# buaacyw/MeshAnything

Measured on NVIDIA H100. Metric: face-tokens/sec (350M, 800-face cap), higher is better.
Workload: dtype f16 weights/activations, f32 accumulate

## Files before the change

### meshanything_b200/csrc/api.cu

```cuda
#include <stdarg.h>
#include <stdlib.h>
#include <stdio.h>
#include <string.h>

#include <atomic>
#include <map>
#include <mutex>
#include <vector>

#include "canon.cuh"
#include "internal.h"

namespace ma {

static thread_local char g_err[512] = "";
static std::atomic<unsigned long long> g_launches{0};

void set_error(const char* fmt, ...) {
  va_list ap;
  va_start(ap, fmt);
  vsnprintf(g_err, sizeof(g_err), fmt, ap);
  va_end(ap);
}
void count_launch(int n) { g_launches += (unsigned long long)n; }
bool check_launch(const char* what) {
  cudaError_t e = cudaPeekAtLastError();
  if (e != cudaSuccess) {
    set_error("%s: %s", what, cudaGetErrorString(e));
    cudaGetLastError();
    return false;
  }
  return true;
}

static inline size_t align_up(size_t x, size_t a = 256) { return (x + a - 1) / a * a; }

constexpr int PREFILL_SEQS = 8;

struct DecWs {
  float* hres;
  __half *x16, *qkv, *attn16, *y16, *f16, *logits, *lastx16;
  int* nkeys;
  SeqState s;
  int* all_done;
  void* attn_scratch;
  size_t attn_scratch_bytes;
  void* attn_scratch_pre;
  size_t attn_scratch_pre_bytes;
  void* fast;
  void* tc_scratch;
  size_t total;
};

static DecWs carve(void* base, int B, int tmax, int vocab) {
  DecWs w;
  const size_t rows = (size_t)std::max(B, PREFIX * std::min(B, PREFILL_SEQS));
  size_t off = 0;
  auto take = [&](size_t bytes) {
    void* p = base ? (void*)((char*)base + off) : nullptr;
    off += align_up(bytes);
    return p;
  };
  w.hres = (float*)take(rows * HID * 4);
  w.x16 = (__half*)take(rows * HID * 2);
  w.qkv = (__half*)take(rows * QKV * 2);
  w.attn16 = (__half*)take(rows * HID * 2);
  w.y16 = (__half*)take(rows * HID * 2);
  w.f16 = (__half*)take(rows * FFN * 2);
  w.logits = (__half*)take((size_t)B * vocab * 2);
  w.lastx16 = (__half*)take((size_t)B * HID * 2);
  w.nkeys = (int*)take(rows * 4);
  w.s.pos = (int*)take((size_t)B * 4);
  w.s.gen = (int*)take((size_t)B * 4);
  w.s.tok = (int*)take((size_t)B * 4);
  w.s.finished = (int*)take((size_t)B * 4);
  w.s.lens = (int*)take((size_t)B * 4);
  w.s.sid = (int*)take((size_t)B * 4);
  w.all_done = (int*)take(256);
  w.attn_scratch_bytes = attention_scratch_bytes((int)B, NHEAD, tmax);
  w.attn_scratch = take(w.attn_scratch_bytes);
  w.attn_scratch_pre_bytes = attention_scratch_bytes(PREFIX * std::min(B, PREFILL_SEQS), NHEAD, PREFIX);
  w.attn_scratch_pre = take(w.attn_scratch_pre_bytes);
  w.fast = take(fast_workspace_bytes());
  w.tc_scratch = take(linear_ws_scratch_bytes());
  w.total = off;
  return w;
}

static inline __half* kv_layer(void* kv, int layer, int which, int B, long T) {
  return (__half*)kv + ((size_t)(layer * 2 + which) * B) * NHEAD * T * HD;
}

static const bool g_no_stream_attn = [] {
  const char* e = getenv("MA_B200_NO_STREAM_ATTN");
  return e && e[0] == '1';
}();

static const bool g_no_pdl = [] {
  const char* e = getenv("MA_B200_NO_PDL");
  return e && e[0] == '1';
}();

static int dec_linear(bool tc, const DecWs& ws, const void* W, const void* b, const __half* x, int ldx, __half* y, int ldy,
                      int M, int N, int K, int epi, cudaStream_t st, bool pdl = false) {
  if (tc) {
    const bool tiled_ok = M >= 64 && linear_tc_supported(M, N, K, ldx, ldy, x, W, y);
    const bool ws_ok = M <= 128 && linear_ws_supported(M, N, K, ldx, x, W);
    if (ws_ok && (linear_ws_mode() || !tiled_ok || K > 1024))
      return launch_linear_ws((const __half*)W, (const __half*)b, x, ldx, y, ldy, M, N, K, epi, ws.tc_scratch, st, pdl);
    if (tiled_ok) return launch_linear_tc((const __half*)W, (const __half*)b, x, ldx, y, ldy, M, N, K, epi, st);
  }
  return launch_linear((const __half*)W, (const __half*)b, x, ldx, y, ldy, M, N, K, epi, st);
}

static int run_layers(const ma_decoder_weights* w, const DecWs& ws, void* kv, int B, long T, int M, int rows_per_slot,
                      int slot0, int max_keys, cudaStream_t st, bool tc = false) {
  void* scratch = rows_per_slot > 1 ? ws.attn_scratch_pre : ws.attn_scratch;
  const bool pdl = tc && rows_per_slot == 1 && !g_no_pdl;
  for (int L = 0; L < w->n_layers; L++) {
    __half* kc = kv_layer(kv, L, 0, B, T) + (size_t)slot0 * NHEAD * T * HD;
    __half* vc = kv_layer(kv, L, 1, B, T) + (size_t)slot0 * NHEAD * T * HD;
    if (dec_linear(tc, ws, w->wqkv[L], w->bqkv[L], ws.x16, HID, ws.qkv, QKV, M, QKV, HID, MA_EPI_NONE, st, pdl)) return 1;
    if (rows_per_slot == 1 && !g_no_stream_attn) {
      if (launch_attention_decode(ws.qkv, QKV, kc, vc, T, ws.nkeys, max_keys, M, 0.125f, ws.attn16, HID, scratch, pdl,
                                  st)) return 1;
    } else {
      if (launch_kv_append(ws.qkv, M, rows_per_slot, ws.nkeys, kc, vc, T, st)) return 1;
      if (launch_attention(ws.qkv, QKV, kc, vc, T, NHEAD, rows_per_slot, nullptr, ws.nkeys, max_keys, M, 0.125f,
                           ws.attn16, HID, scratch, st)) return 1;
    }
    if (dec_linear(tc, ws, w->wo[L], w->bo[L], ws.attn16, HID, ws.y16, HID, M, HID, HID, MA_EPI_NONE, st, pdl)) return 1;
    if (launch_layernorm(ws.hres, ws.y16, w->ln1g[L], w->ln1b[L], MA_LN_EPS, M, HID, ws.hres, ws.x16, st, pdl)) return 1;
    if (dec_linear(tc, ws, w->w1[L], w->b1[L], ws.x16, HID, ws.f16, FFN, M, FFN, HID, MA_EPI_RELU, st, pdl)) return 1;
    if (dec_linear(tc, ws, w->w2[L], w->b2[L], ws.f16, FFN, ws.y16, HID, M, HID, FFN, MA_EPI_NONE, st, pdl)) return 1;
    if (launch_layernorm(ws.hres, ws.y16, w->ln2g[L], w->ln2b[L], MA_LN_EPS, M, HID, ws.hres, ws.x16, st, pdl)) return 1;
  }
  return 0;
}

struct GraphKey {
  const void *w, *kv, *ws, *out_ids, *forced, *logits_out;
  unsigned long long whash;
  int B, tmax, max_new, bucket, flags, do_sample, top_k, eos, pad, mode, ws_mode;
  float top_p;
  unsigned long long seed;
  bool operator<(const GraphKey& o) const { return memcmp(this, &o, sizeof(GraphKey)) < 0; }
};
static std::map<GraphKey, cudaGraphExec_t> g_graphs;
static std::map<cudaGraphExec_t, unsigned long long> g_graph_launches;
static cudaStream_t g_stream = nullptr;
static int* g_flag_host = nullptr;
static cudaEvent_t g_ev_in = nullptr, g_ev_out = nullptr, g_ev_flag = nullptr;

static int g_device = -1;
static std::mutex g_mu;

static int ensure_globals() {
  int dev = -1;
  if (cudaGetDevice(&dev) != cudaSuccess) {
    set_error("cudaGetDevice: %s", cudaGetErrorString(cudaGetLastError()));
    return 1;
  }
  if (g_device >= 0 && dev != g_device) {
    set_error("ma_decode_generate was first used on device %d; this process now runs on device %d "
              "(one process per GPU)", g_device, dev);
    return 1;
  }
  if (!g_stream) {
    if (cudaStreamCreateWithFlags(&g_stream, cudaStreamNonBlocking) != cudaSuccess ||
        cudaHostAlloc((void**)&g_flag_host, 64, cudaHostAllocDefault) != cudaSuccess ||
        cudaEventCreateWithFlags(&g_ev_in, cudaEventDisableTiming) != cudaSuccess ||
        cudaEventCreateWithFlags(&g_ev_out, cudaEventDisableTiming) != cudaSuccess ||
        cudaEventCreateWithFlags(&g_ev_flag, cudaEventDisableTiming) != cudaSuccess) {
      set_error("cannot create stream/events: %s", cudaGetErrorString(cudaGetLastError()));
      return 1;
    }
    g_device = dev;
  }
  return 0;
}


static int enqueue_batched_step(const ma_decoder_weights* w, const DecWs& ws, void* kv, int B, long T, int max_keys,
                                const SampleArgs& sa, cudaStream_t s, bool tc) {
  if (launch_embed_tokens(w, ws.s, B, ws.hres, ws.x16, ws.nkeys, s)) return 1;
  if (run_layers(w, ws, kv, B, T, B, 1, 0, max_keys, s, tc)) return 1;
  if (dec_linear(tc, ws, w->lm_head, nullptr, ws.x16, HID, ws.logits, w->vocab, B, w->vocab, HID, MA_EPI_NONE, s,
                 tc && !g_no_pdl)) return 1;
  return launch_sample(sa, s);
}

static inline bool use_tc(int B, int do_sample, int flags) { return B > 1 && (do_sample || (flags & MA_GEN_TC)); }

static unsigned long long weights_hash(const ma_decoder_weights* w) {
  unsigned long long h = 1469598103934665603ull;
  const unsigned char* pb = (const unsigned char*)w;
  for (size_t q = 0; q < sizeof(ma_decoder_weights); q++) h = (h ^ pb[q]) * 1099511628211ull;
  return h;
}

template <class F>
static int launch_cached_graph(const GraphKey& key, cudaStream_t st, F&& enqueue) {
  auto it = g_graphs.find(key);
  if (it == g_graphs.end()) {
    cudaGraph_t graph = nullptr;
    if (cudaStreamBeginCapture(st, cudaStreamCaptureModeThreadLocal) != cudaSuccess) {
      set_error("cudaStreamBeginCapture: %s", cudaGetErrorString(cudaGetLastError()));
      return 1;
    }
    const unsigned long long before = g_launches.load();
    int erc = enqueue(st);
    const unsigned long long per_step = g_launches.load() - before;
    cudaError_t ce = cudaStreamEndCapture(st, &graph);
    if (erc || ce != cudaSuccess || !graph) {
      if (!erc) set_error("cudaStreamEndCapture: %s", cudaGetErrorString(ce));
      cudaGetLastError();
      return 1;
    }
    cudaGraphExec_t exec = nullptr;
    ce = cudaGraphInstantiate(&exec, graph, 0);
    cudaGraphDestroy(graph);
    if (ce != cudaSuccess) {
      set_error("cudaGraphInstantiate: %s", cudaGetErrorString(ce));
      return 1;
    }
    if (g_graphs.size() > 64) {
      for (auto& kvp : g_graphs) cudaGraphExecDestroy(kvp.second);
      g_graphs.clear();
      g_graph_launches.clear();
    }
    it = g_graphs.emplace(key, exec).first;
    g_launches -= per_step;
    g_graph_launches[exec] = per_step;
  }
  if (cudaGraphLaunch(it->second, st) != cudaSuccess) {
    set_error("cudaGraphLaunch: %s", cudaGetErrorString(cudaGetLastError()));
    return 1;
  }
  g_launches += g_graph_launches[it->second];
  return 0;
}

static void fill_sample_args(SampleArgs& sa, const ma_decoder_weights* w, const DecWs& ws, int B, int max_new,
                             const ma_sampling* sampling, int eos_id, int pad_id, int32_t* out_ids) {
  memset(&sa, 0, sizeof(sa));
  sa.logits = ws.logits; sa.vocab = w->vocab; sa.B = B; sa.max_new = max_new; sa.eos_id = eos_id; sa.pad_id = pad_id;
  sa.do_sample = sampling ? sampling->do_sample : 0;
  sa.top_k = sampling ? sampling->top_k : 0;
  sa.top_p = sampling ? sampling->top_p : 1.0f;
  sa.seed = sampling ? sampling->seed : 0;
  sa.s = ws.s; sa.out_ids = out_ids;
}

static int check_decode_args(const char* who, const ma_decoder_weights* w, int B, int tmax, int max_new) {
  if (w->n_layers > MA_MAX_LAYERS || w->vocab > 8195 + 61) {
    set_error("%s: n_layers=%d / vocab=%d unsupported", who, w->n_layers, w->vocab);
    return 1;
  }
  if (B <= 0 || max_new <= 0 || PREFIX + max_new > tmax) {
    set_error("%s: B=%d, tmax=%d < 257 + max_new=%d", who, B, tmax, max_new);
    return 1;
  }
  if (PREFIX + max_new + 2 > w->npos) {
    set_error("%s: sequence of %d exceeds %d learned positions", who, PREFIX + max_new, w->npos - 2);
    return 1;
  }
  return 0;
}

}

using namespace ma;

extern "C" {

int ma_abi_version(void) { return MA_ABI_VERSION; }
const char* ma_last_error(void) { return g_err; }
unsigned long long ma_launch_count(void) { return g_launches.load(); }

int ma_linear_f16(const void* W, const void* bias, const void* x, int ldx, void* y, int ldy, int M, int N, int K,
                  int epilogue, void* stream) {
  return launch_linear((const __half*)W, (const __half*)bias, (const __half*)x, ldx, (__half*)y, ldy, M, N, K,
                       epilogue, (cudaStream_t)stream);
}

size_t ma_linear_ws_scratch_bytes(void) { return linear_ws_scratch_bytes(); }
void ma_linear_ws_set_mode(int cluster) { linear_ws_set_mode(cluster); }

int ma_linear_ws_f16(const void* W, const void* bias, const void* x, int ldx, void* y, int ldy, int M, int N, int K,
                     int epilogue, void* scratch, void* stream) {
  return launch_linear_ws((const __half*)W, (const __half*)bias, (const __half*)x, ldx, (__half*)y, ldy, M, N, K,
                          epilogue, scratch, (cudaStream_t)stream);
}

int ma_layernorm(const float* x, const void* res16, const float* gamma, const float* beta, float eps, int M, int W,
                 float* out32, void* out16, void* stream) {
  return launch_layernorm(x, (const __half*)res16, gamma, beta, eps, M, W, out32, (__half*)out16,
                          (cudaStream_t)stream);
}

size_t ma_attention_scratch_bytes(int M, int H, int max_keys) { return attention_scratch_bytes(M, H, max_keys); }

int ma_attention_f16(const void* q, int ldq, const void* K, const void* V, long T, int H, const int* slots,
                     const int* nkeys, int max_keys, int M, float scale, void* out, int ldo, void* scratch,
                     void* stream) {
  if (M > 65535) {
    set_error("ma_attention_f16: M=%d exceeds 65535 rows per call", M);
    return 1;
  }
  return launch_attention((const __half*)q, ldq, (const __half*)K, (const __half*)V, T, H, 1, slots, nkeys, max_keys, M,
                          scale, (__half*)out, ldo, scratch, (cudaStream_t)stream);
}

int ma_attention_decode_f16(const void* qkv, int ldq, void* K, void* V, long T, const int* nkeys, int max_keys, int M,
                            float scale, void* out, int ldo, void* scratch, void* stream) {
  if (!qkv || !K || !V || !nkeys || !out || !scratch || M < 1 || max_keys < 1 || max_keys > T || ldq < 3 * HID) {
    set_error("ma_attention_decode_f16: bad arguments (M=%d, max_keys=%d, T=%ld, ldq=%d)", M, max_keys, T, ldq);
    return 1;
  }
  return launch_attention_decode((const __half*)qkv, ldq, (__half*)K, (__half*)V, T, nkeys, max_keys, M, scale,
                                 (__half*)out, ldo, scratch, false, (cudaStream_t)stream);
}

int ma_sample_tokens(const void* logits, int B, int vocab, const ma_sampling* sampling, int32_t* out_tokens,
                     int32_t* out_support, void* stream) {
  if (!logits || !out_tokens || B < 1 || vocab < 1) {
    set_error("ma_sample_tokens: bad arguments");
    return 1;
  }
  SampleArgs sa;
  memset(&sa, 0, sizeof(sa));
  sa.logits = (const __half*)logits; sa.vocab = vocab; sa.B = B; sa.max_new = 1; sa.eos_id = -1; sa.pad_id = -1;
  sa.do_sample = sampling ? sampling->do_sample : 0;
  sa.top_k = sampling ? sampling->top_k : 0;
  sa.top_p = sampling ? sampling->top_p : 1.0f;
  sa.seed = sampling ? sampling->seed : 0;
  sa.first = 1; sa.token_out = out_tokens; sa.support_out = out_support;
  return launch_sample(sa, (cudaStream_t)stream);
}

size_t ma_kv_cache_bytes(int n_layers, int B, int tmax) {
  return (size_t)n_layers * 2 * B * NHEAD * (size_t)tmax * HD * sizeof(__half);
}

size_t ma_decoder_workspace_bytes(int B, int tmax) { return carve(nullptr, B, tmax, 8195 + 61).total; }

int ma_decode_generate(const ma_decoder_weights* w, const float* prefix, int B, int tmax, int max_new,
                       const ma_sampling* sampling, int eos_id, int pad_id, void* kv, void* ws_, int32_t* out_ids,
                       int32_t* out_lens, const int32_t* forced_ids, void* logits_out, int flags, void* stream) {
  if (!w || !prefix || !kv || !ws_ || !out_ids || B <= 0 || max_new <= 0) {
    set_error("ma_decode_generate: bad arguments");
    return 1;
  }
  if (check_decode_args("ma_decode_generate", w, B, tmax, max_new)) return 1;
  std::lock_guard<std::mutex> lock(g_mu);
  if (ensure_globals()) return 1;
  cudaStream_t user = (cudaStream_t)stream;
  cudaStream_t st = g_stream;
  cudaEventRecord(g_ev_in, user);
  cudaStreamWaitEvent(st, g_ev_in, 0);

  const long T = tmax;
  DecWs ws = carve(ws_, B, tmax, 8195 + 61);
  cudaMemsetAsync(ws.attn_scratch, 0, ws.attn_scratch_bytes, st);
  cudaMemsetAsync(ws.attn_scratch_pre, 0, ws.attn_scratch_pre_bytes, st);
  cudaMemsetAsync(ws.fast, 0, fast_workspace_bytes(), st);
  if (launch_fill_i32(out_ids, pad_id, (long)B * max_new, st)) return 1;

  SampleArgs sa;
  fill_sample_args(sa, w, ws, B, max_new, sampling, eos_id, pad_id, out_ids);
  sa.first = 1; sa.forced = forced_ids; sa.logits_out = (__half*)logits_out;
  sa.all_done = ws.all_done;

  const bool tc = use_tc(B, sa.do_sample, flags);
  if (tc) cudaMemsetAsync(ws.tc_scratch, 0, linear_ws_scratch_bytes(), st);
  const bool fast = (B == 1) && !(flags & MA_GEN_NO_FAST);
  if (fast) sa.nkeys_next = fast_nkeys_ptr(ws.fast);

  for (int b0 = 0; b0 < B; b0 += PREFILL_SEQS) {
    const int nb = std::min(PREFILL_SEQS, B - b0), M = nb * PREFIX;
    if (launch_embed_prefix(w, prefix + (size_t)b0 * PREFIX * HID, nb, ws.hres, ws.x16, ws.nkeys, st)) return 1;
    if (run_layers(w, ws, kv, B, T, M, PREFIX, b0, PREFIX, st, tc)) return 1;
    if (launch_gather_rows(ws.x16, HID, PREFIX - 1, PREFIX, nb, ws.lastx16 + (size_t)b0 * HID, st)) return 1;
  }
  if (dec_linear(tc, ws, w->lm_head, nullptr, ws.lastx16, HID, ws.logits, w->vocab, B, w->vocab, HID, MA_EPI_NONE, st))
    return 1;
  if (launch_sample(sa, st)) return 1;
  sa.first = 0;
  sa.nkeys_next = nullptr;


  const bool use_graph = !(flags & MA_GEN_NO_GRAPH);
  const bool early = !(flags & MA_GEN_NO_EARLY_EXIT) && !forced_ids;
  const int CHECK_EVERY = 64;
  const unsigned long long whash = use_graph ? weights_hash(w) : 0;
  bool flag_pending = false;
  int rc = 0;
  for (int i = 1; i < max_new && rc == 0; i++) {
    const int ctx = PREFIX + i;
// ... 193 lines not shown
```

### meshanything_b200/csrc/attention_stream.cu

```cuda
#include "canon.cuh"
#include "internal.h"

namespace ma {

constexpr int AS_SLOTS = 3;
constexpr int AS_TEAM = 256;
constexpr int AS_THREADS = 32 + AS_TEAM;
constexpr int AS_PART = 66;
constexpr int AS_MERGE_BLOCK = 29;

struct AttnStreamSmem {
  __half ring[AS_SLOTS][MA_ATTN_CHUNK * HD];
  float red[8][65];
  float pst[AS_MERGE_BLOCK * AS_PART];
  float wgt[64];
  float mst[64];
  float wmax[8];
  uint64_t full[AS_SLOTS], empty[AS_SLOTS];
  int last;
};
static_assert(2 * (sizeof(AttnStreamSmem) + 1024) <= 233472, "two CTAs of attention_stream_kernel per SM");

struct AttnStreamArgs {
  const __half* q;
  int ldq;
  __half* K;
  __half* V;
  long T;
  const int* nkeys;
  __half* out;
  int ldo;
  float* part;
  int* counters;
  int M, max_chunks;
  int cps, nseg;
  float scale;
};

__device__ __forceinline__ void team_bar() { asm volatile("bar.sync 1, %0;" ::"n"(AS_TEAM) : "memory"); }
__device__ __forceinline__ void mbar_arrive(uint64_t* bar) {
  asm volatile("mbarrier.arrive.shared::cta.b64 _, [%0];" ::"r"(smem_u32(bar)) : "memory");
}

struct AsItem {
  int m, h, c0, c1, n, nk, nch;
};
__device__ __forceinline__ bool as_item(const AttnStreamArgs& a, int w, AsItem& it) {
  const int g = w % a.nseg, h = (w / a.nseg) % NHEAD;
  it.m = w / (a.nseg * NHEAD);
  it.h = h;
  it.nk = __ldcg(a.nkeys + it.m);
  it.n = min(it.nk, a.max_chunks * MA_ATTN_CHUNK);
  it.nch = (it.n + MA_ATTN_CHUNK - 1) / MA_ATTN_CHUNK;
  it.c0 = g * a.cps;
  it.c1 = min(it.nch, it.c0 + a.cps);
  return it.c0 < it.c1;
}

__global__ void __launch_bounds__(AS_THREADS, 2) attention_stream_kernel(AttnStreamArgs a) {
  extern __shared__ __align__(128) unsigned char smem_raw[];
  AttnStreamSmem& sm = *reinterpret_cast<AttnStreamSmem*>(smem_raw);
  const int tid = threadIdx.x, warp = tid >> 5, lane = tid & 31;
  const int nitems = a.nseg * NHEAD * a.M;

  if (tid == 0) {
    for (int s = 0; s < AS_SLOTS; s++) {
      mbar_init(&sm.full[s], 1);
      mbar_init(&sm.empty[s], 1);
    }
    mbar_fence_init();
  }
  __syncthreads();

  if (warp == 0) {
    if (lane != 0) return;
    int u = 0;
    for (int w = blockIdx.x; w < nitems; w += gridDim.x) {
      AsItem it;
      if (!as_item(a, w, it)) continue;
      for (int c = it.c0; c < it.c1; c++) {
        const int len = min(MA_ATTN_CHUNK, it.n - c * MA_ATTN_CHUNK);
        const int old = (it.nk == it.n) ? min(len, (it.n - 1) - c * MA_ATTN_CHUNK) : len;
        const long base = (((long)it.m * NHEAD + it.h) * a.T + (long)c * MA_ATTN_CHUNK) * HD;
#pragma unroll
        for (int kv = 0; kv < 2; kv++, u++) {
          const int s = u % AS_SLOTS;
          if (u >= AS_SLOTS) mbar_wait(&sm.empty[s], ((u / AS_SLOTS) & 1) ^ 1);
          if (old > 0) {
            mbar_expect_tx(&sm.full[s], (uint32_t)old * HD * 2);
            bulk_g2s(sm.ring[s], (kv ? a.V : a.K) + base, (uint32_t)old * HD * 2, &sm.full[s]);
          } else {
            mbar_arrive(&sm.full[s]);
          }
        }
      }
    }
    return;
  }

  const int wt = warp - 1, tl = tid - 32;
  const int grp = lane >> 3, li = lane & 7;
  pdl_wait();
  pdl_trigger();
  int u = 0;
  for (int w = blockIdx.x; w < nitems; w += gridDim.x) {
    AsItem it;
    if (!as_item(a, w, it)) continue;
    const int m = it.m, h = it.h, nch = it.nch;
    const __half* qrow = a.q + (long)m * a.ldq + h * HD + 8 * li;
    const uint4 qp = *reinterpret_cast<const uint4*>(qrow);
    float* part = a.part + (((long)m * NHEAD + h) * a.max_chunks) * AS_PART;

    for (int c = it.c0; c < it.c1; c++, u += 2) {
      const int sk = u % AS_SLOTS, sv = (u + 1) % AS_SLOTS;
      const int len = min(MA_ATTN_CHUNK, it.n - c * MA_ATTN_CHUNK);
      const int cur = (it.nk == it.n) ? (it.n - 1) - c * MA_ATTN_CHUNK : -1;
      uint4 kcur = make_uint4(0, 0, 0, 0), vcur = kcur;
      const bool own_cur = cur >= 0 && cur < MA_ATTN_CHUNK && (4 * wt + grp) == (cur & 31);
      if (own_cur) {
        kcur = *reinterpret_cast<const uint4*>(qrow + HID);
        vcur = *reinterpret_cast<const uint4*>(qrow + 2 * HID);
        const long dst = (((long)m * NHEAD + h) * a.T + (long)c * MA_ATTN_CHUNK + cur) * HD + 8 * li;
        *reinterpret_cast<uint4*>(a.K + dst) = kcur;
        *reinterpret_cast<uint4*>(a.V + dst) = vcur;
      }
      const int rho_c = own_cur ? (cur >> 5) : -1;
      const __half* ks = sm.ring[sk];
      const __half* vs = sm.ring[sv];
      mbar_wait(&sm.full[sk], (u / AS_SLOTS) & 1);

      float pr[8];
#pragma unroll
      for (int rho = 0; rho < 8; rho++) {
        const int r = 32 * rho + 4 * wt + grp;
        uint4 x = *reinterpret_cast<const uint4*>(ks + r * HD + 8 * li);
        if (rho == rho_c) x = kcur;
        pr[rho] = dot8(qp, x, 0.0f);
      }
#pragma unroll
      for (int sft = 4; sft >= 1; sft >>= 1) {
        const bool up = (li & sft) != 0;
#pragma unroll
        for (int t = 0; t < sft; t++) {
          const float mine = up ? pr[t + sft] : pr[t];
          const float other = up ? pr[t] : pr[t + sft];
          pr[t] = fadd(mine, __shfl_xor_sync(0xffffffffu, other, sft));
        }
      }
      const float s_own = fmul(pr[0], a.scale);
      const bool own_valid = 32 * li + 4 * wt + grp < len;
      const float lmax = warp_max(own_valid ? s_own : -INFINITY);
      if (lane == 0) sm.wmax[wt] = lmax;
      team_bar();
      if (tl == 0) mbar_arrive(&sm.empty[sk]);
      float cmax = sm.wmax[0];
#pragma unroll
      for (int w2 = 1; w2 < 8; w2++) cmax = fmaxf(cmax, sm.wmax[w2]);
      const float e_own = own_valid ? ma_exp(fsub(s_own, cmax)) : 0.0f;
      float l = 0.0f, o[8];
#pragma unroll
      for (int t = 0; t < 8; t++) o[t] = 0.0f;
      mbar_wait(&sm.full[sv], ((u + 1) / AS_SLOTS) & 1);
#pragma unroll
      for (int rho = 0; rho < 8; rho++) {
        const int r = 32 * rho + 4 * wt + grp;
        const float e = __shfl_sync(0xffffffffu, e_own, (lane & 24) | rho);
        if (r < len) {
          l = fadd(l, e);
          uint4 x = *reinterpret_cast<const uint4*>(vs + r * HD + 8 * li);
          if (rho == rho_c) x = vcur;
          pv8(__float2half_rn(e), x, o);
        }
      }
      l = fadd(l, __shfl_xor_sync(0xffffffffu, l, 16));
      l = fadd(l, __shfl_xor_sync(0xffffffffu, l, 8));
#pragma unroll
      for (int t = 0; t < 8; t++) {
        o[t] = fadd(o[t], __shfl_xor_sync(0xffffffffu, o[t], 16));
        o[t] = fadd(o[t], __shfl_xor_sync(0xffffffffu, o[t], 8));
      }
      if (grp == 0) {
#pragma unroll
        for (int t = 0; t < 8; t++) sm.red[wt][8 * li + t] = o[t];
        if (li == 0) sm.red[wt][64] = l;
      }
      team_bar();
      if (tl == 0) mbar_arrive(&sm.empty[sv]);
      if (tl < 65) {
        float x[8];
#pragma unroll
        for (int w2 = 0; w2 < 8; w2++) x[w2] = sm.red[w2][tl];
        const float rsum = fadd(fadd(fadd(x[0], x[1]), fadd(x[2], x[3])), fadd(fadd(x[4], x[5]), fadd(x[6], x[7])));
        if (nch == 1) {
          sm.pst[tl] = rsum;
        } else {
          part[c * AS_PART + (tl < 64 ? tl : 65)] = rsum;
          if (tl == 64) part[c * AS_PART + 64] = cmax;
        }
      }
    }

    if (nch == 1) {
      team_bar();
      if (tl < 64) a.out[(long)m * a.ldo + h * HD + tl] = __float2half_rn(__fdiv_rn(sm.pst[tl], sm.pst[64]));
      team_bar();
      continue;
    }
    __threadfence();
    team_bar();
    const int nseg_row = (nch + a.cps - 1) / a.cps;
    if (nseg_row > 1) {
      if (tl == 0) {
        int* cnt = a.counters + (long)m * NHEAD + h;
        const int prev = atomicAdd(cnt, 1);
        const int last = (prev == nseg_row - 1);
        if (last) *cnt = 0;
        sm.last = last;
      }
      team_bar();
      const int last = sm.last;
      team_bar();
      if (!last) continue;
      __threadfence();
    }
    const bool single = nch <= AS_MERGE_BLOCK;
    if (!single) {
      for (int t = tl; t < nch; t += AS_TEAM) sm.mst[t] = __ldcg(part + t * AS_PART + 64);
      team_bar();
      float Mx = -INFINITY;
      for (int cc = 0; cc < nch; cc++) Mx = fmaxf(Mx, sm.mst[cc]);
      for (int t = tl; t < nch; t += AS_TEAM) sm.wgt[t] = ma_exp(fsub(sm.mst[t], Mx));
    }
    float Lsum = 0.0f, O = 0.0f;
    for (int c0 = 0; c0 < nch; c0 += AS_MERGE_BLOCK) {
      const int nb = min(AS_MERGE_BLOCK, nch - c0), nw = nb * AS_PART;
      for (int t = tl; t < nw; t += AS_TEAM) sm.pst[t] = __ldcg(part + (long)c0 * AS_PART + t);
      team_bar();
      if (single) {
        float Mx = -INFINITY;
        for (int cc = 0; cc < nch; cc++) Mx = fmaxf(Mx, sm.pst[cc * AS_PART + 64]);
        for (int t = tl; t < nch; t += AS_TEAM) sm.wgt[t] = ma_exp(fsub(sm.pst[t * AS_PART + 64], Mx));
        team_bar();
      }
      if (tl < 64) {
        for (int cc = 0; cc < nb; cc++) {
          const float wc = sm.wgt[c0 + cc];
          Lsum = ffma(sm.pst[cc * AS_PART + 65], wc, Lsum);
          O = ffma(sm.pst[cc * AS_PART + tl], wc, O);
        }
      }
      team_bar();
    }
    if (tl < 64) a.out[(long)m * a.ldo + h * HD + tl] = __float2half_rn(__fdiv_rn(O, Lsum));
  }
}

static int g_as_ctas = 0;

int launch_attention_decode(const __half* qkv, int ldq, __half* K, __half* V, long T, const int* nkeys, int max_keys,
                            int M, float scale, __half* out, int ldo, void* scratch, bool pdl, cudaStream_t st) {
  if (M <= 0) return 0;
  if (!g_as_ctas) {
    int dev = 0, sms = 0;
    cudaGetDevice(&dev);
    cudaDeviceGetAttribute(&sms, cudaDevAttrMultiProcessorCount, dev);
    cudaFuncSetAttribute(attention_stream_kernel, cudaFuncAttributeMaxDynamicSharedMemorySize,
                         (int)sizeof(AttnStreamSmem));
    g_as_ctas = 2 * (sms > 0 ? sms : 132);
  }
  const int chunks = (max_keys + MA_ATTN_CHUNK - 1) / MA_ATTN_CHUNK;
  AttnStreamArgs a;
  a.q = qkv; a.ldq = ldq; a.K = K; a.V = V; a.T = T; a.nkeys = nkeys; a.out = out; a.ldo = ldo;
  a.counters = reinterpret_cast<int*>(scratch);
  const size_t coff = ((size_t)M * NHEAD * sizeof(int) + 255) & ~(size_t)255;
  a.part = reinterpret_cast<float*>(reinterpret_cast<char*>(scratch) + coff);
  a.M = M; a.max_chunks = chunks; a.scale = scale;
  {
    long best = -1;
    int best_cps = 1;
    for (int cps = 1; cps <= chunks; cps++) {
      const int nseg = (chunks + cps - 1) / cps;
      const long items = (long)nseg * NHEAD * M;
      const long cost = ((items + g_as_ctas - 1) / g_as_ctas) * (long)(min(cps, chunks) + 1);
      if (best < 0 || cost <= best) { best = cost; best_cps = cps; }
    }
    a.cps = best_cps;
    a.nseg = (chunks + a.cps - 1) / a.cps;
  }
  const long nitems = (long)a.nseg * NHEAD * M;
  cudaLaunchConfig_t cfg = {};
  cfg.gridDim = dim3((unsigned)min((long)g_as_ctas, nitems));
  cfg.blockDim = dim3(AS_THREADS);
  cfg.dynamicSmemBytes = sizeof(AttnStreamSmem);
  cfg.stream = st;
  cudaLaunchAttribute at[1];
  at[0].id = cudaLaunchAttributeProgrammaticStreamSerialization;
  at[0].val.programmaticStreamSerializationAllowed = 1;
  cfg.attrs = at;
  cfg.numAttrs = pdl ? 1 : 0;
  cudaLaunchKernelEx(&cfg, attention_stream_kernel, a);
  count_launch();
  return check_launch("attention_stream_kernel") ? 0 : 1;
}

}
```

### meshanything_b200/csrc/decode_fast.cu

```cuda
#include "canon.cuh"
#include "internal.h"

namespace ma {

int launch_attention_ex(const __half* q, int ldq, const __half* K, const __half* V, long T, int H, int rows_per_slot,
                        const int* slots, const int* nkeys, int max_keys, int M, float scale, __half* out, int ldo,
                        void* scratch, int decode_prefetch, bool pdl, cudaStream_t st);

constexpr int FG_THREADS = 256;
constexpr int FG_WARPS = 8;

enum { MODE_QKV = 0, MODE_OUT = 1, MODE_FC1 = 2, MODE_FC2 = 3, MODE_LM = 4 };

struct FastWs {
  float hresA[HID];
  float hresB[HID];
  __half q[HID];
  __half attn16[HID];
  __half y16[HID];
  __half f16[FFN];
  __half logits[8256];
  float cand_val[256];
  int cand_idx[256];
  int counter;
  int nkeys;
  alignas(256) unsigned char attn_scratch[256];
};

struct FastArgs {
  const __half* W;
  const __half* bias;
  int N, rows_per_cta;
  const float* hres_in;
  const __half* y16_in;
  const float *gamma, *beta;
  const __half* x16_in;
  float* hres_out;
  int embed;
  const float *extra, *tok_pos, *cond, *pos_table;
  const __half* tok_table;
  SeqState s;
  __half* out16;
  __half *kc, *vc;
  long T;
  FastWs* ws;
  int do_argmax;
  int max_new, eos_id, pad_id;
  int32_t* out_ids;
  const int32_t* forced;
  __half* logits_out;
  int* all_done;
  int vocab;
};

template <int K>
struct alignas(128) FastSmemHdr {
  uint64_t bar[FG_WARPS];
  float red[8];
  float bval[FG_WARPS];
  int bidx[FG_WARPS];
  int last;
  alignas(16) __half xs[K];
};

template <int K, int MODE>
__global__ void __launch_bounds__(FG_THREADS) fast_gemv_kernel(FastArgs a) {
  extern __shared__ __align__(128) unsigned char smem_raw[];
  FastSmemHdr<K>& sh = *reinterpret_cast<FastSmemHdr<K>*>(smem_raw);
  __half* sw = reinterpret_cast<__half*>(smem_raw + sizeof(FastSmemHdr<K>));
  __half* sb = sw + (size_t)a.rows_per_cta * K;
  const int tid = threadIdx.x, warp = tid >> 5, lane = tid & 31;

  if (MODE != MODE_QKV) pdl_trigger();

  const int row0 = blockIdx.x * a.rows_per_cta;
  const int nrows = max(0, min(a.rows_per_cta, a.N - row0));
  const int base = nrows / FG_WARPS, rem = nrows % FG_WARPS;
  const int wr0 = warp * base + min(warp, rem);
  const int wn = base + (warp < rem ? 1 : 0);

  if (lane == 0) {
    mbar_init(&sh.bar[warp], 1);
    mbar_fence_init();
  }
  __syncwarp();
  if (lane == 0 && wn > 0) {
    mbar_expect_tx(&sh.bar[warp], (uint32_t)wn * K * 2);
    bulk_g2s(sw + (size_t)wr0 * K, a.W + (size_t)(row0 + wr0) * K, (uint32_t)wn * K * 2, &sh.bar[warp]);
  }
  if (a.bias)
    for (int i = tid; i < nrows; i += FG_THREADS) sb[i] = a.bias[row0 + i];
  float4 ln_g, ln_b, cond;
  if (MODE == MODE_QKV && a.embed) {
    cond = *reinterpret_cast<const float4*>(a.cond + HID + 4 * tid);
  } else if (MODE == MODE_QKV || MODE == MODE_FC1 || MODE == MODE_LM) {
    ln_g = *reinterpret_cast<const float4*>(a.gamma + 4 * tid);
    ln_b = *reinterpret_cast<const float4*>(a.beta + 4 * tid);
  }

  pdl_wait();
  if (MODE == MODE_QKV) pdl_trigger();

  if (MODE == MODE_QKV || MODE == MODE_FC1 || MODE == MODE_LM) {
    float v[4];
    if (MODE == MODE_QKV && a.embed) {
      const int tok = a.s.tok[0], gen = a.s.gen[0], pos = a.s.pos[0];
      float4 X;
      int fidx;
      if (tok < 3) {
        X = *reinterpret_cast<const float4*>(a.extra + (long)tok * HID + 4 * tid);
        fidx = tok;
      } else {
        const uint2 u = *reinterpret_cast<const uint2*>(a.tok_table + (long)(tok - 3) * HID + 4 * tid);
        const __half2* h = reinterpret_cast<const __half2*>(&u);
        const float2 p0 = __half22float2(h[0]), p1 = __half22float2(h[1]);
        X = make_float4(p0.x, p0.y, p1.x, p1.y);
        int r = (gen - 2) % 9;
        if (r < 0) r += 9;
        fidx = r + 3;
      }
      const float4 F = *reinterpret_cast<const float4*>(a.tok_pos + (long)fidx * HID + 4 * tid);
      const float4 C = cond;
      const float4 P = *reinterpret_cast<const float4*>(a.pos_table + (long)(pos + 2) * HID + 4 * tid);
      v[0] = fadd(fadd(fadd(X.x, F.x), C.x), P.x);
      v[1] = fadd(fadd(fadd(X.y, F.y), C.y), P.y);
      v[2] = fadd(fadd(fadd(X.z, F.z), C.z), P.z);
      v[3] = fadd(fadd(fadd(X.w, F.w), C.w), P.w);
    } else {
      const float4 hv = *reinterpret_cast<const float4*>(a.hres_in + 4 * tid);
      const uint2 u = *reinterpret_cast<const uint2*>(a.y16_in + 4 * tid);
      const __half2* h = reinterpret_cast<const __half2*>(&u);
      const float2 p0 = __half22float2(h[0]), p1 = __half22float2(h[1]);
      v[0] = fadd(hv.x, p0.x); v[1] = fadd(hv.y, p0.y); v[2] = fadd(hv.z, p1.x); v[3] = fadd(hv.w, p1.y);
      layernorm4(v, ln_g, ln_b, MA_LN_EPS, HID, sh.red);
    }
    if (blockIdx.x == 0 && a.hres_out)
      *reinterpret_cast<float4*>(a.hres_out + 4 * tid) = make_float4(v[0], v[1], v[2], v[3]);
    __half2 h0 = __floats2half2_rn(v[0], v[1]), h1 = __floats2half2_rn(v[2], v[3]);
    uint2 u;
    u.x = *reinterpret_cast<uint32_t*>(&h0);
    u.y = *reinterpret_cast<uint32_t*>(&h1);
    *reinterpret_cast<uint2*>(sh.xs + 4 * tid) = u;
  } else {
    for (int i = tid; i < K / 8; i += FG_THREADS)
      *reinterpret_cast<uint4*>(sh.xs + 8 * i) = *reinterpret_cast<const uint4*>(a.x16_in + 8 * i);
  }
  __syncthreads();

  constexpr int G = K / 256;
  uint4 xp[G];
#pragma unroll
  for (int g = 0; g < G; g++) xp[g] = *reinterpret_cast<const uint4*>(sh.xs + 256 * g + 8 * lane);

  int pos = 0;
  if (MODE == MODE_QKV) pos = a.s.pos[0];
  float bestv = -INFINITY;
  int besti = 0x7fffffff;

  if (wn > 0) mbar_wait(&sh.bar[warp], 0);
  constexpr int RB = (K == HID) ? 4 : 1;
  for (int r0 = 0; r0 < wn; r0 += RB) {
    float acc[RB];
#pragma unroll
    for (int i = 0; i < RB; i++) acc[i] = 0.0f;
#pragma unroll
    for (int g = 0; g < G; g++) {
      float xf[8];
      unpack8(xp[g], xf);
#pragma unroll
      for (int i = 0; i < RB; i++) {
        const int r = min(r0 + i, wn - 1);
        const uint4 u = *reinterpret_cast<const uint4*>(sw + (size_t)(wr0 + r) * K + 256 * g + 8 * lane);
        float wf[8];
        unpack8(u, wf);
#pragma unroll
        for (int j = 0; j < 8; j++) acc[i] = ffma(wf[j], xf[j], acc[i]);
      }
    }
#pragma unroll
    for (int i = 0; i < RB; i++) {
      const float sum = warp_sum(acc[i]);
      const int n = row0 + wr0 + r0 + i;
      if (r0 + i < wn && lane == 0) {
        const float bf = a.bias ? __half2float(sb[wr0 + r0 + i]) : 0.0f;
        __half h = __float2half_rn(fadd(sum, bf));
        if (MODE == MODE_FC1 && __half2float(h) < 0.0f) h = __float2half_rn(0.0f);
        if (MODE == MODE_QKV) {
          if (n < HID) {
            a.out16[n] = h;
          } else {
            const int e = (n - HID) & (HID - 1), head = e >> 6, d = e & 63;
            __half* c = (n < 2 * HID) ? a.kc : a.vc;
            c[((long)head * a.T + pos) * HD + d] = h;
          }
        } else {
          a.out16[n] = h;
        }
        if (MODE == MODE_LM) {
          const float v = __half2float(h);
          if (v > bestv || (v == bestv && n < besti)) { bestv = v; besti = n; }
        }
      }
    }
  }

  if (MODE == MODE_LM) {
    FastWs* ws = a.ws;
    const int gen = a.s.gen[0];
    if (a.logits_out) {
      __syncthreads();
      for (int i = tid; i < nrows; i += FG_THREADS)
        a.logits_out[(long)gen * a.vocab + row0 + i] = a.out16[row0 + i];
    }
    if (!a.do_argmax) return;
    if (lane == 0) { sh.bval[warp] = bestv; sh.bidx[warp] = besti; }
    __syncthreads();
    if (tid == 0) {
      float bv = sh.bval[0];
      int bi = sh.bidx[0];
      for (int w = 1; w < FG_WARPS; w++)
        if (sh.bval[w] > bv || (sh.bval[w] == bv && sh.bidx[w] < bi)) { bv = sh.bval[w]; bi = sh.bidx[w]; }
      ws->cand_val[blockIdx.x] = bv;
      ws->cand_idx[blockIdx.x] = bi;
      __threadfence();
      const int prev = atomicAdd(&ws->counter, 1);
      sh.last = (prev == (int)gridDim.x - 1);
      if (sh.last) ws->counter = 0;
    }
    __syncthreads();
    if (!sh.last) return;
    __threadfence();
    float bv = -INFINITY;
    int bi = 0x7fffffff;
    for (int i = tid; i < (int)gridDim.x; i += FG_THREADS) {
      const float v = __ldcg(&ws->cand_val[i]);
      const int ix = __ldcg(&ws->cand_idx[i]);
      if (v > bv || (v == bv && ix < bi)) { bv = v; bi = ix; }
    }
#pragma unroll
    for (int o = 16; o > 0; o >>= 1) {
      const float ov = __shfl_xor_sync(0xffffffffu, bv, o);
      const int oi = __shfl_xor_sync(0xffffffffu, bi, o);
      if (ov > bv || (ov == bv && oi < bi)) { bv = ov; bi = oi; }
    }
    if (lane == 0) { sh.bval[warp] = bv; sh.bidx[warp] = bi; }
    __syncthreads();
    if (tid == 0) {
      for (int w = 1; w < FG_WARPS; w++)
        if (sh.bval[w] > bv || (sh.bval[w] == bv && sh.bidx[w] < bi)) { bv = sh.bval[w]; bi = sh.bidx[w]; }
      int tok = bi;
      if (a.forced) tok = a.forced[gen];
      int fin = a.s.finished[0];
      if (fin) tok = a.pad_id;
      if (gen < a.max_new) a.out_ids[gen] = tok;
      if (!fin) a.s.lens[0] = gen + 1;
      if (!fin && tok == a.eos_id) fin = 1;
      a.s.finished[0] = fin;
      a.s.tok[0] = tok;
      a.s.gen[0] = gen + 1;
      const int np = a.s.pos[0] + 1;
      a.s.pos[0] = np;
      ws->nkeys = np + 1;
      if (a.all_done) *a.all_done = fin;
    }
  }
}

static int g_sms = 0;

size_t fast_workspace_bytes() {
  return sizeof(FastWs) + attention_scratch_bytes(1, NHEAD, 18432) + 256;
}

template <int K, int MODE>
static int launch_fast(const FastArgs& a, int grid, bool pdl, cudaStream_t st) {
  const size_t smem = sizeof(FastSmemHdr<K>) + (size_t)a.rows_per_cta * K * 2 + (((size_t)a.rows_per_cta * 2 + 15) & ~(size_t)15);
  static size_t attr_set = 0;
  if (smem > attr_set) {
    cudaFuncSetAttribute(fast_gemv_kernel<K, MODE>, cudaFuncAttributeMaxDynamicSharedMemorySize, (int)smem);
    attr_set = smem;
  }
  cudaLaunchConfig_t cfg = {};
  cfg.gridDim = dim3(grid);
  cfg.blockDim = dim3(FG_THREADS);
  cfg.dynamicSmemBytes = smem;
  cfg.stream = st;
  cudaLaunchAttribute at[1];
  at[0].id = cudaLaunchAttributeProgrammaticStreamSerialization;
  at[0].val.programmaticStreamSerializationAllowed = 1;
  cfg.attrs = at;
  cfg.numAttrs = pdl ? 1 : 0;
  cudaLaunchKernelEx(&cfg, fast_gemv_kernel<K, MODE>, a);
  count_launch();
  return check_launch("fast_gemv_kernel") ? 0 : 1;
}

int fast_step_enqueue(const ma_decoder_weights* w, SeqState s, int tmax, int max_keys, __half* kv, void* fast_ws,
                      const SampleArgs& sa, bool pdl, cudaStream_t st) {
  if (!g_sms) {
    int dev = 0;
    cudaGetDevice(&dev);
    cudaDeviceGetAttribute(&g_sms, cudaDevAttrMultiProcessorCount, dev);
    if (g_sms <= 0 || g_sms > 256) g_sms = 132;
  }
  const int grid = g_sms;
  FastWs* ws = reinterpret_cast<FastWs*>(fast_ws);
  const long T = tmax;
  auto rpc = [&](int N) { return (N + grid - 1) / grid; };

  FastArgs base;
  memset(&base, 0, sizeof(base));
  base.s = s;
  base.T = T;
  base.ws = ws;
  base.extra = w->extra; base.tok_pos = w->tok_pos; base.cond = w->cond; base.pos_table = w->pos;
  base.tok_table = (const __half*)w->tok_table;
  base.vocab = w->vocab;

  for (int L = 0; L < w->n_layers; L++) {
    __half* kc = kv + ((size_t)(L * 2 + 0)) * NHEAD * T * HD;
    __half* vc = kv + ((size_t)(L * 2 + 1)) * NHEAD * T * HD;
    {
      FastArgs a = base;
      a.W = (const __half*)w->wqkv[L]; a.bias = (const __half*)w->bqkv[L]; a.N = QKV; a.rows_per_cta = rpc(QKV);
      a.embed = (L == 0);
      if (L > 0) { a.hres_in = ws->hresB; a.y16_in = ws->y16; a.gamma = w->ln2g[L - 1]; a.beta = w->ln2b[L - 1]; }
      a.hres_out = ws->hresA;
      a.out16 = ws->q; a.kc = kc; a.vc = vc;
      if (launch_fast<HID, MODE_QKV>(a, grid, pdl, st)) return 1;
    }
    if (launch_attention_ex(ws->q, HID, kc, vc, T, NHEAD, 1, nullptr, &ws->nkeys, max_keys, 1, 0.125f, ws->attn16, HID,
                            ws->attn_scratch, 1, pdl, st)) return 1;
    {
      FastArgs a = base;
      a.W = (const __half*)w->wo[L]; a.bias = (const __half*)w->bo[L]; a.N = HID; a.rows_per_cta = rpc(HID);
      a.x16_in = ws->attn16; a.out16 = ws->y16;
      if (launch_fast<HID, MODE_OUT>(a, grid, pdl, st)) return 1;
    }
    {
      FastArgs a = base;
      a.W = (const __half*)w->w1[L]; a.bias = (const __half*)w->b1[L]; a.N = FFN; a.rows_per_cta = rpc(FFN);
      a.hres_in = ws->hresA; a.y16_in = ws->y16; a.gamma = w->ln1g[L]; a.beta = w->ln1b[L];
      a.hres_out = ws->hresB; a.out16 = ws->f16;
      if (launch_fast<HID, MODE_FC1>(a, grid, pdl, st)) return 1;
    }
    {
      FastArgs a = base;
      a.W = (const __half*)w->w2[L]; a.bias = (const __half*)w->b2[L]; a.N = HID; a.rows_per_cta = rpc(HID);
      a.x16_in = ws->f16; a.out16 = ws->y16;
      if (launch_fast<FFN, MODE_FC2>(a, grid, pdl, st)) return 1;
    }
  }
  {
    FastArgs a = base;
    const int L = w->n_layers - 1;
    a.W = (const __half*)w->lm_head; a.bias = nullptr; a.N = w->vocab; a.rows_per_cta = rpc(w->vocab);
    a.hres_in = ws->hresB; a.y16_in = ws->y16; a.gamma = w->ln2g[L]; a.beta = w->ln2b[L];
    a.out16 = sa.do_sample ? const_cast<__half*>(sa.logits) : ws->logits;
    a.do_argmax = !sa.do_sample;
    a.max_new = sa.max_new; a.eos_id = sa.eos_id; a.pad_id = sa.pad_id;
    a.out_ids = sa.out_ids; a.forced = sa.forced; a.logits_out = sa.logits_out; a.all_done = sa.all_done;
    if (launch_fast<HID, MODE_LM>(a, grid, pdl, st)) return 1;
  }
  if (sa.do_sample) {
    SampleArgs s2 = sa;
    s2.logits_out = nullptr;
    s2.nkeys_next = &ws->nkeys;
    if (launch_sample(s2, st)) return 1;
  }
  return 0;
}

int* fast_nkeys_ptr(void* fast_ws) { return &reinterpret_cast<FastWs*>(fast_ws)->nkeys; }

}
```

### meshanything_b200/csrc/internal.h

```cpp
#pragma once
#include <cuda_fp16.h>
#include <cuda_runtime.h>
#include <stdint.h>

#include "../../include/meshanything_b200.h"

namespace ma {

constexpr int HID = 1024;
constexpr int NHEAD = 16;
constexpr int HD = 64;
constexpr int FFN = 4096;
constexpr int PREFIX = 257;
constexpr int QKV = 3 * HID;

struct SeqState {
  int* pos;
  int* gen;
  int* tok;
  int* finished;
  int* lens;
  int* sid;
};

void set_error(const char* fmt, ...);
void count_launch(int n = 1);
bool check_launch(const char* what);

int launch_linear(const __half* W, const __half* bias, const __half* x, int ldx, __half* y, int ldy, int M, int N,
                  int K, int epi, cudaStream_t st);

bool attention_tc_supported(int ldq, int ldo, long T, long Tpad, int nkeys, const void* q, const void* K, const void* Vt,
                            const void* out);
int launch_attention_tc(const __half* q, int ldq, const __half* K, const __half* Vt, long T, long Tpad, int H,
                        int rows_per_slot, int n_slots, int nkeys, float scale, __half* out, int ldo, cudaStream_t st);
int launch_scatter_heads_t(const __half* src, int ld, int col0, int head_stride, int H, int n, long Tpad, int n_slots,
                           __half* dst, cudaStream_t st);

bool linear_tc_supported(int M, int N, int K, int ldx, int ldy, const void* x, const void* W, const void* y);
int launch_linear_tc(const __half* W, const __half* bias, const __half* x, int ldx, __half* y, int ldy, int M, int N,
                     int K, int epi, cudaStream_t st);

size_t linear_ws_scratch_bytes();
void linear_ws_set_mode(int cluster);
int linear_ws_mode();
bool linear_ws_supported(int M, int N, int K, int ldx, const void* x, const void* W);
int launch_linear_ws(const __half* W, const __half* bias, const __half* x, int ldx, __half* y, int ldy, int M, int N,
                     int K, int epi, void* scratch, cudaStream_t st, bool pdl = false);

size_t attention_scratch_bytes(int M, int H, int max_keys);
int launch_attention_decode(const __half* qkv, int ldq, __half* K, __half* V, long T, const int* nkeys, int max_keys,
                            int M, float scale, __half* out, int ldo, void* scratch, bool pdl, cudaStream_t st);
int launch_attention(const __half* q, int ldq, const __half* K, const __half* V, long T, int H, int rows_per_slot,
                     const int* slots, const int* nkeys, int max_keys, int M, float scale, __half* out, int ldo,
                     void* scratch, cudaStream_t st);

int launch_layernorm(const float* x, const __half* res16, const float* gamma, const float* beta, float eps, int M,
                     int W, float* out32, __half* out16, cudaStream_t st, bool pdl = false);
int launch_embed_prefix(const ma_decoder_weights* w, const float* prefix, int B, float* hres, __half* x16, int* nkeys,
                        cudaStream_t st);
int launch_embed_tokens(const ma_decoder_weights* w, SeqState s, int B, float* hres, __half* x16, int* nkeys,
                        cudaStream_t st);
int launch_kv_append(const __half* qkv, int M, int rows_per_slot, const int* nkeys, __half* kc, __half* vc, long T,
                     cudaStream_t st);
int launch_gather_rows(const __half* src, int ld, int row0, int stride, int B, __half* dst, cudaStream_t st);
struct SampleArgs {
  const __half* logits;
  int vocab, B, max_new, eos_id, pad_id;
  int do_sample, top_k;
  float top_p;
  unsigned long long seed;
  SeqState s;
  int first;
  int32_t* out_ids;
  const int32_t* forced;
  __half* logits_out;
  int* all_done;
  int* nkeys_next;
  int32_t* support_out;
  int32_t* token_out;
  int row0, nrows;
  int slots;
};
int launch_sample(const SampleArgs& a, cudaStream_t st);
int launch_fill_i32(int32_t* p, int v, long n, cudaStream_t st);

int* fast_nkeys_ptr(void* fast_ws);
size_t fast_workspace_bytes();
int fast_step_enqueue(const ma_decoder_weights* w, SeqState s, int tmax, int max_keys, __half* kv, void* fast_ws,
                      const SampleArgs& sa, bool pdl, cudaStream_t st);

}
```

Measured before the change: 1466.

## Route single-row fast decode through streaming attention with fused KV append

The single-sequence fast decode path now writes the full QKV vector to a workspace and calls the TMA-streamed attention kernel, which appends the current K/V row itself, instead of having the QKV GEMV scatter K/V into the cache and then running the older attention kernel. The streaming kernel is templated on ring depth, using a 4-slot ring with one CTA per SM for M==1, sized so it can sit alongside the out_proj and fc1 GEMV CTAs. It also caches each row's nkeys load and prefetches it before the PDL wait. The aim is less scattered KV writing in the GEMV epilogue and deeper prefetch for the single-row case, at the cost of halving the attention CTA count for that case.

```diff
diff --git a/meshanything_b200/csrc/api.cu b/meshanything_b200/csrc/api.cu
--- a/meshanything_b200/csrc/api.cu
+++ b/meshanything_b200/csrc/api.cu
@@ -95,6 +95,7 @@
   const char* e = getenv("MA_B200_NO_STREAM_ATTN");
   return e && e[0] == '1';
 }();
+bool no_stream_attn() { return g_no_stream_attn; }
 
 static const bool g_no_pdl = [] {
   const char* e = getenv("MA_B200_NO_PDL");
diff --git a/meshanything_b200/csrc/attention_stream.cu b/meshanything_b200/csrc/attention_stream.cu
--- a/meshanything_b200/csrc/attention_stream.cu
+++ b/meshanything_b200/csrc/attention_stream.cu
@@ -3,23 +3,28 @@
 
 namespace ma {
 
-constexpr int AS_SLOTS = 3;
+constexpr int AS_SLOTS_BATCH = 3;
+constexpr int AS_SLOTS_ROW = 4;
 constexpr int AS_TEAM = 256;
 constexpr int AS_THREADS = 32 + AS_TEAM;
 constexpr int AS_PART = 66;
 constexpr int AS_MERGE_BLOCK = 29;
 
+template <int SLOTS>
 struct AttnStreamSmem {
-  __half ring[AS_SLOTS][MA_ATTN_CHUNK * HD];
+  __half ring[SLOTS][MA_ATTN_CHUNK * HD];
   float red[8][65];
   float pst[AS_MERGE_BLOCK * AS_PART];
   float wgt[64];
   float mst[64];
   float wmax[8];
-  uint64_t full[AS_SLOTS], empty[AS_SLOTS];
+  uint64_t full[SLOTS], empty[SLOTS];
   int last;
 };
-static_assert(2 * (sizeof(AttnStreamSmem) + 1024) <= 233472, "two CTAs of attention_stream_kernel per SM");
+static_assert(2 * (sizeof(AttnStreamSmem<AS_SLOTS_BATCH>) + 1024) <= 233472, "two CTAs of the batch geometry per SM");
+static_assert(sizeof(AttnStreamSmem<AS_SLOTS_ROW>) + 1024 + (18704 + 1024) + (67904 + 1024) <= 233472 &&
+                  2 * (sizeof(AttnStreamSmem<AS_SLOTS_ROW>) + 1024) > 233472,
+              "one CTA of the single-row geometry per SM, co-resident with the out_proj and fc1 GEMV CTAs");
 
 struct AttnStreamArgs {
   const __half* q;
@@ -45,11 +50,20 @@
 struct AsItem {
   int m, h, c0, c1, n, nk, nch;
 };
-__device__ __forceinline__ bool as_item(const AttnStreamArgs& a, int w, AsItem& it) {
+__device__ __forceinline__ int as_row(const AttnStreamArgs& a, int w) { return w / (a.nseg * NHEAD); }
+__device__ __forceinline__ int as_nkeys(const AttnStreamArgs& a, int w, int& row, int& nk) {
+  const int m = as_row(a, w);
+  if (m != row) {
+    row = m;
+    nk = __ldcg(a.nkeys + m);
+  }
+  return nk;
+}
+__device__ __forceinline__ bool as_item(const AttnStreamArgs& a, int w, int nk, AsItem& it) {
   const int g = w % a.nseg, h = (w / a.nseg) % NHEAD;
-  it.m = w / (a.nseg * NHEAD);
+  it.m = as_row(a, w);
   it.h = h;
-  it.nk = __ldcg(a.nkeys + it.m);
+  it.nk = nk;
   it.n = min(it.nk, a.max_chunks * MA_ATTN_CHUNK);
   it.nch = (it.n + MA_ATTN_CHUNK - 1) / MA_ATTN_CHUNK;
   it.c0 = g * a.cps;
@@ -57,14 +71,15 @@
   return it.c0 < it.c1;
 }
 
+template <int SLOTS>
 __global__ void __launch_bounds__(AS_THREADS, 2) attention_stream_kernel(AttnStreamArgs a) {
   extern __shared__ __align__(128) unsigned char smem_raw[];
-  AttnStreamSmem& sm = *reinterpret_cast<AttnStreamSmem*>(smem_raw);
+  AttnStreamSmem<SLOTS>& sm = *reinterpret_cast<AttnStreamSmem<SLOTS>*>(smem_raw);
   const int tid = threadIdx.x, warp = tid >> 5, lane = tid & 31;
   const int nitems = a.nseg * NHEAD * a.M;
 
   if (tid == 0) {
-    for (int s = 0; s < AS_SLOTS; s++) {
+    for (int s = 0; s < SLOTS; s++) {
       mbar_init(&sm.full[s], 1);
       mbar_init(&sm.empty[s], 1);
     }
@@ -74,18 +89,18 @@
 
   if (warp == 0) {
     if (lane != 0) return;
-    int u = 0;
+    int u = 0, row = -1, nk = 0;
     for (int w = blockIdx.x; w < nitems; w += gridDim.x) {
       AsItem it;
-      if (!as_item(a, w, it)) continue;
+      if (!as_item(a, w, as_nkeys(a, w, row, nk), it)) continue;
       for (int c = it.c0; c < it.c1; c++) {
         const int len = min(MA_ATTN_CHUNK, it.n - c * MA_ATTN_CHUNK);
         const int old = (it.nk == it.n) ? min(len, (it.n - 1) - c * MA_ATTN_CHUNK) : len;
         const long base = (((long)it.m * NHEAD + it.h) * a.T + (long)c * MA_ATTN_CHUNK) * HD;
 #pragma unroll
         for (int kv = 0; kv < 2; kv++, u++) {
-          const int s = u % AS_SLOTS;
-          if (u >= AS_SLOTS) mbar_wait(&sm.empty[s], ((u / AS_SLOTS) & 1) ^ 1);
+          const int s = u % SLOTS;
+          if (u >= SLOTS) mbar_wait(&sm.empty[s], ((u / SLOTS) & 1) ^ 1);
           if (old > 0) {
             mbar_expect_tx(&sm.full[s], (uint32_t)old * HD * 2);
             bulk_g2s(sm.ring[s], (kv ? a.V : a.K) + base, (uint32_t)old * HD * 2, &sm.full[s]);
@@ -100,19 +115,21 @@
 
   const int wt = warp - 1, tl = tid - 32;
   const int grp = lane >> 3, li = lane & 7;
+  int row = -1, nk = 0;
+  if (blockIdx.x < nitems) as_nkeys(a, blockIdx.x, row, nk);
   pdl_wait();
   pdl_trigger();
   int u = 0;
   for (int w = blockIdx.x; w < nitems; w += gridDim.x) {
     AsItem it;
-    if (!as_item(a, w, it)) continue;
+    if (!as_item(a, w, as_nkeys(a, w, row, nk), it)) continue;
     const int m = it.m, h = it.h, nch = it.nch;
     const __half* qrow = a.q + (long)m * a.ldq + h * HD + 8 * li;
     const uint4 qp = *reinterpret_cast<const uint4*>(qrow);
     float* part = a.part + (((long)m * NHEAD + h) * a.max_chunks) * AS_PART;
 
     for (int c = it.c0; c < it.c1; c++, u += 2) {
-      const int sk = u % AS_SLOTS, sv = (u + 1) % AS_SLOTS;
+      const int sk = u % SLOTS, sv = (u + 1) % SLOTS;
       const int len = min(MA_ATTN_CHUNK, it.n - c * MA_ATTN_CHUNK);
       const int cur = (it.nk == it.n) ? (it.n - 1) - c * MA_ATTN_CHUNK : -1;
       uint4 kcur = make_uint4(0, 0, 0, 0), vcur = kcur;
@@ -127,7 +144,7 @@
       const int rho_c = own_cur ? (cur >> 5) : -1;
       const __half* ks = sm.ring[sk];
       const __half* vs = sm.ring[sv];
-      mbar_wait(&sm.full[sk], (u / AS_SLOTS) & 1);
+      mbar_wait(&sm.full[sk], (u / SLOTS) & 1);
 
       float pr[8];
 #pragma unroll
@@ -160,7 +177,7 @@
       float l = 0.0f, o[8];
 #pragma unroll
       for (int t = 0; t < 8; t++) o[t] = 0.0f;
-      mbar_wait(&sm.full[sv], ((u + 1) / AS_SLOTS) & 1);
+      mbar_wait(&sm.full[sv], ((u + 1) / SLOTS) & 1);
 #pragma unroll
       for (int rho = 0; rho < 8; rho++) {
         const int r = 32 * rho + 4 * wt + grp;
@@ -255,19 +272,23 @@
   }
 }
 
-static int g_as_ctas = 0;
+static int g_as_sms = 0;
 
 int launch_attention_decode(const __half* qkv, int ldq, __half* K, __half* V, long T, const int* nkeys, int max_keys,
                             int M, float scale, __half* out, int ldo, void* scratch, bool pdl, cudaStream_t st) {
   if (M <= 0) return 0;
-  if (!g_as_ctas) {
+  if (!g_as_sms) {
     int dev = 0, sms = 0;
     cudaGetDevice(&dev);
     cudaDeviceGetAttribute(&sms, cudaDevAttrMultiProcessorCount, dev);
-    cudaFuncSetAttribute(attention_stream_kernel, cudaFuncAttributeMaxDynamicSharedMemorySize,
-                         (int)sizeof(AttnStreamSmem));
-    g_as_ctas = 2 * (sms > 0 ? sms : 132);
-  }
+    cudaFuncSetAttribute(attention_stream_kernel<AS_SLOTS_BATCH>, cudaFuncAttributeMaxDynamicSharedMemorySize,
+                         (int)sizeof(AttnStreamSmem<AS_SLOTS_BATCH>));
+    cudaFuncSetAttribute(attention_stream_kernel<AS_SLOTS_ROW>, cudaFuncAttributeMaxDynamicSharedMemorySize,
+                         (int)sizeof(AttnStreamSmem<AS_SLOTS_ROW>));
+    g_as_sms = sms > 0 ? sms : 132;
+  }
+  const bool row = M == 1;
+  const int ctas = (row ? 1 : 2) * g_as_sms;
   const int chunks = (max_keys + MA_ATTN_CHUNK - 1) / MA_ATTN_CHUNK;
   AttnStreamArgs a;
   a.q = qkv; a.ldq = ldq; a.K = K; a.V = V; a.T = T; a.nkeys = nkeys; a.out = out; a.ldo = ldo;
@@ -281,7 +302,7 @@
     for (int cps = 1; cps <= chunks; cps++) {
       const int nseg = (chunks + cps - 1) / cps;
       const long items = (long)nseg * NHEAD * M;
-      const long cost = ((items + g_as_ctas - 1) / g_as_ctas) * (long)(min(cps, chunks) + 1);
+      const long cost = ((items + ctas - 1) / ctas) * (long)(min(cps, chunks) + 1);
       if (best < 0 || cost <= best) { best = cost; best_cps = cps; }
     }
     a.cps = best_cps;
@@ -289,16 +310,19 @@
   }
   const long nitems = (long)a.nseg * NHEAD * M;
   cudaLaunchConfig_t cfg = {};
-  cfg.gridDim = dim3((unsigned)min((long)g_as_ctas, nitems));
+  cfg.gridDim = dim3((unsigned)min((long)ctas, nitems));
   cfg.blockDim = dim3(AS_THREADS);
-  cfg.dynamicSmemBytes = sizeof(AttnStreamSmem);
+  cfg.dynamicSmemBytes = row ? sizeof(AttnStreamSmem<AS_SLOTS_ROW>) : sizeof(AttnStreamSmem<AS_SLOTS_BATCH>);
   cfg.stream = st;
   cudaLaunchAttribute at[1];
   at[0].id = cudaLaunchAttributeProgrammaticStreamSerialization;
   at[0].val.programmaticStreamSerializationAllowed = 1;
   cfg.attrs = at;
   cfg.numAttrs = pdl ? 1 : 0;
-  cudaLaunchKernelEx(&cfg, attention_stream_kernel, a);
+  if (row)
+    cudaLaunchKernelEx(&cfg, attention_stream_kernel<AS_SLOTS_ROW>, a);
+  else
+    cudaLaunchKernelEx(&cfg, attention_stream_kernel<AS_SLOTS_BATCH>, a);
   count_launch();
   return check_launch("attention_stream_kernel") ? 0 : 1;
 }
diff --git a/meshanything_b200/csrc/decode_fast.cu b/meshanything_b200/csrc/decode_fast.cu
--- a/meshanything_b200/csrc/decode_fast.cu
+++ b/meshanything_b200/csrc/decode_fast.cu
@@ -15,7 +15,7 @@
 struct FastWs {
   float hresA[HID];
   float hresB[HID];
-  __half q[HID];
+  __half qkv[QKV];
   __half attn16[HID];
   __half y16[HID];
   __half f16[FFN];
@@ -41,8 +41,6 @@
   const __half* tok_table;
   SeqState s;
   __half* out16;
-  __half *kc, *vc;
-  long T;
   FastWs* ws;
   int do_argmax;
   int max_new, eos_id, pad_id;
@@ -152,8 +150,6 @@
 #pragma unroll
   for (int g = 0; g < G; g++) xp[g] = *reinterpret_cast<const uint4*>(sh.xs + 256 * g + 8 * lane);
 
-  int pos = 0;
-  if (MODE == MODE_QKV) pos = a.s.pos[0];
   float bestv = -INFINITY;
   int besti = 0x7fffffff;
 
@@ -185,17 +181,7 @@
         const float bf = a.bias ? __half2float(sb[wr0 + r0 + i]) : 0.0f;
         __half h = __float2half_rn(fadd(sum, bf));
         if (MODE == MODE_FC1 && __half2float(h) < 0.0f) h = __float2half_rn(0.0f);
-        if (MODE == MODE_QKV) {
-          if (n < HID) {
-            a.out16[n] = h;
-          } else {
-            const int e = (n - HID) & (HID - 1), head = e >> 6, d = e & 63;
-            __half* c = (n < 2 * HID) ? a.kc : a.vc;
-            c[((long)head * a.T + pos) * HD + d] = h;
-          }
-        } else {
-          a.out16[n] = h;
-        }
+        a.out16[n] = h;
         if (MODE == MODE_LM) {
           const float v = __half2float(h);
           if (v > bestv || (v == bestv && n < besti)) { bestv = v; besti = n; }
@@ -311,7 +297,6 @@
   FastArgs base;
   memset(&base, 0, sizeof(base));
   base.s = s;
-  base.T = T;
   base.ws = ws;
   base.extra = w->extra; base.tok_pos = w->tok_pos; base.cond = w->cond; base.pos_table = w->pos;
   base.tok_table = (const __half*)w->tok_table;
@@ -326,11 +311,17 @@
       a.embed = (L == 0);
       if (L > 0) { a.hres_in = ws->hresB; a.y16_in = ws->y16; a.gamma = w->ln2g[L - 1]; a.beta = w->ln2b[L - 1]; }
       a.hres_out = ws->hresA;
-      a.out16 = ws->q; a.kc = kc; a.vc = vc;
+      a.out16 = ws->qkv;
       if (launch_fast<HID, MODE_QKV>(a, grid, pdl, st)) return 1;
     }
-    if (launch_attention_ex(ws->q, HID, kc, vc, T, NHEAD, 1, nullptr, &ws->nkeys, max_keys, 1, 0.125f, ws->attn16, HID,
-                            ws->attn_scratch, 1, pdl, st)) return 1;
+    if (!no_stream_attn()) {
+      if (launch_attention_decode(ws->qkv, QKV, kc, vc, T, &ws->nkeys, max_keys, 1, 0.125f, ws->attn16, HID,
+                                  ws->attn_scratch, pdl, st)) return 1;
+    } else {
+      if (launch_kv_append(ws->qkv, 1, 1, &ws->nkeys, kc, vc, T, st)) return 1;
+      if (launch_attention_ex(ws->qkv, QKV, kc, vc, T, NHEAD, 1, nullptr, &ws->nkeys, max_keys, 1, 0.125f, ws->attn16,
+                              HID, ws->attn_scratch, 1, pdl, st)) return 1;
+    }
     {
       FastArgs a = base;
       a.W = (const __half*)w->wo[L]; a.bias = (const __half*)w->bo[L]; a.N = HID; a.rows_per_cta = rpc(HID);
diff --git a/meshanything_b200/csrc/internal.h b/meshanything_b200/csrc/internal.h
--- a/meshanything_b200/csrc/internal.h
+++ b/meshanything_b200/csrc/internal.h
@@ -54,6 +54,7 @@
 int launch_attention(const __half* q, int ldq, const __half* K, const __half* V, long T, int H, int rows_per_slot,
                      const int* slots, const int* nkeys, int max_keys, int M, float scale, __half* out, int ldo,
                      void* scratch, cudaStream_t st);
+bool no_stream_attn();
 
 int launch_layernorm(const float* x, const __half* res16, const float* gamma, const float* beta, float eps, int M,
                      int W, float* out32, __half* out16, cudaStream_t st, bool pdl = false);
```

After: 1569 (median of 6 runs). +7.0%, better.
